# hanseongbugi/ORB_SLAM3_Study_kr

Hardware: AMD Instinct MI355X
Metric: local-BA windows/sec (50 KF, 10k pts, 10 LM iters) + ORB matches/sec; 1/2/4/8 GPU (higher is better)
Workload: dtype f64; 1 GPU; BASELINE.json configs[1]: synthetic stereo local BA, 50 optimisable + 10 fixed KF, 10k landmarks (~75k stereo edges), optimize(10) with the reference's stop rules; windows_per_gpu=512, global_windows=512, streams_per_gpu=2, parallelism=independent windows, w mod 1

## Files before the change

orb_slam3_study_kr_amd/csrc/lba_device.hip:

```cpp
#include <cstdlib>
#include <cstdio>
#include <atomic>
#include <chrono>
#include <thread>
#include "lba_lm_kernels.h"
#include "lba_schur_items.h"
#include "lba_reduce_solve.h"
#include "solve_plan.h"
#include "lba_pack_device.h"
#include <algorithm>
#include <cstring>
#include <vector>

using namespace osh;

namespace osh {

constexpr int kDevicePackMinWindows = 24;

__global__ __launch_bounds__(256) void k_gather_out(BatchView bv, const int* lm_perm, int n_points_total, double* out_pose, double* out_pts,
                                                    const int* pt_win) {
  const int t = blockIdx.x * blockDim.x + threadIdx.x;
  if (t < n_points_total) {
    const int w = pt_win[t];
// ... 26 lines not shown
}

struct osh_lba_ctx {
  int device = 0;
  hipStream_t stream = nullptr;
  void* attach[kAttachCount] = {};
  void (*attach_free[kAttachCount])(void*) = {};
  KernelTimer timer;
  int n_windows = 0;
  PackedBatch pb;
  std::vector<const volatile unsigned char*> stop_ptr;
  bool any_stop = false;
  int solve_nb = 24, solve_W = 0, solve_threads = kSolveThreadsLatency;
  bool solve_big = false;
  DevBuf d_bigV, d_bigz, d_bigfail;
  size_t solve_lds = 0, backsub_lds = 0, lin_lds = 0;
  double upload_pack_ms = 0, upload_copy_ms = 0;
  void (*kp_lin_lm)(BatchView) = nullptr;
  void (*kp_schur_sym)(BatchView, int, int) = nullptr;
  void (*kp_schur_cross)(BatchView, int, int) = nullptr;
  void (*kp_finalize)(BatchView) = nullptr;
  void (*kp_backsub)(BatchView) = nullptr;
  void (*kp_debug_hpl)(BatchView, double*) = nullptr;
  PinBuf h_arena[2], h_out;
  DevBuf d_arena[2], d_ptwin, d_erec;
  DevBuf d_lm, d_pose[2], d_pt[2], d_hcontrib, d_chi_lin, d_dmax_lin, d_contrib, d_ccontrib;
  DevBuf d_Hll, d_bl, d_DL, d_Hpp, d_bp, d_S, d_bs, d_xp, d_chi, d_scale, d_dmaxp, d_nactive, d_out_chi2, d_out_depth, d_stop;
  DevBuf d_out_pose, d_out_pts, d_dbg, d_pose_lo;
  int* h_nactive = nullptr;
  unsigned char* h_stop = nullptr;
  size_t h_stop_cap = 0;
  BatchView bv{};
  bool optimized = false;
  DevPackState dpack;
  int pack_mode = -1;
// ... 68 lines not shown
  } else {
    const int rc = pack_batch(nw, pr, [&](int which, size_t bytes) { return c->h_arena[which].reserve(bytes); }, default_pack_threads(nw), cuts, pb);
    if (rc != OSH_OK) { set_error("%s", pb.msg); return rc; }
  }
  const auto t1 = std::chrono::steady_clock::now();
  if (!on_device) {
    for (int a = 0; a < 2; ++a) {
      OSH_TRY(c->d_arena[a].reserve(pb.arena_bytes[a]));
      OSH_HIP(hipMemcpyAsync(c->d_arena[a].p, pb.arena[a], pb.arena_bytes[a], hipMemcpyHostToDevice, s));
    }
  }
  const size_t NP = pb.NP, NFP = pb.NFP, NL = pb.NL, NOUT = pb.NOUT;

  {
    c->lin_lds = (size_t)LinLds::doubles(std::min(pb.np_max, kLdsPoses)) * sizeof(double);
    int backsub_doubles = 0;
    for (const WinDesc& d : pb.win) backsub_doubles = std::max(backsub_doubles, backsub_lds_doubles(d.P, d.F, backsub_stages(d.P, d.F)));
    c->backsub_lds = (size_t)backsub_doubles * sizeof(double);
    auto knob = [](const char* name) { const char* e = std::getenv(name); return e ? std::atoi(e) : 0; };
    const SolvePlan plan = lba_solve_plan(pb.n_max, nw, knob("OSH_LBA_SOLVE_NB"), knob("OSH_LBA_SOLVE_THREADS"), knob("OSH_LBA_SOLVE_BIG"));
    c->solve_threads = plan.threads;
    c->solve_big = plan.big;
    if (c->solve_big) {
      if (pb.n_max / 6 > kBigMaxPoses) {
        set_error("window with %d optimisable poses: the dense reduced system is limited to %d poses", pb.n_max / 6, kBigMaxPoses);
        return OSH_ERR_UNSUPPORTED;
      }
      OSH_TRY(c->d_bigV.reserve(std::max<size_t>((size_t)kBigNB * pb.n_max * 8, 8))); OSH_TRY(c->d_bigz.reserve(std::max<size_t>((size_t)pb.n_max * 8, 8)));
      OSH_TRY(c->d_bigfail.reserve(sizeof(int)));
    }
// ... 9 lines not shown
  OSH_TRY(R(c->d_hcontrib, pb.n_ccontrib * 27 * 8)); OSH_TRY(R(c->d_chi_lin, pb.n_chunks * 8)); OSH_TRY(R(c->d_dmax_lin, pb.n_chunks * 8));
  OSH_TRY(R(c->d_Hll, NL * 6 * 8)); OSH_TRY(R(c->d_bl, NL * 3 * 8)); OSH_TRY(R(c->d_DL, NL * 9 * 8));
  OSH_TRY(R(c->d_Hpp, NFP * 36 * 8)); OSH_TRY(R(c->d_bp, NFP * 6 * 8)); OSH_TRY(R(c->d_S, pb.S_total * 8));
  OSH_TRY(R(c->d_bs, NFP * 6 * 8)); OSH_TRY(R(c->d_xp, NFP * 6 * 8));
  OSH_TRY(R(c->d_chi, pb.n_chunks * 8)); OSH_TRY(R(c->d_scale, pb.n_chunks * 8));
  OSH_TRY(R(c->d_dmaxp, NFP * 8)); OSH_TRY(R(c->d_nactive, sizeof(int)));
  OSH_TRY(R(c->d_out_chi2, NOUT * 8)); OSH_TRY(R(c->d_out_depth, NOUT)); OSH_TRY(R(c->d_stop, nw));
  OSH_TRY(R(c->d_out_pose, NFP * 7 * 8)); OSH_TRY(R(c->d_out_pts, NL * 3 * 8)); OSH_TRY(R(c->d_ptwin, NL * 4)); OSH_TRY(R(c->d_pose_lo, NFP * 4));
  if (c->h_stop_cap < (size_t)nw) {
    if (c->h_stop) (void)hipHostFree(c->h_stop);
    OSH_HIP(hipHostMalloc((void**)&c->h_stop, nw));
    zero_new_host(c->h_stop, nw);
    c->h_stop_cap = nw;
  }
  OSH_HIP(hipMemsetAsync(c->d_xp.p, 0, std::max<size_t>(NFP * 6 * 8, 8), s));
  if (!on_device) {
    int* h_ptwin = static_cast<int*>(c->h_out.reserve(std::max<size_t>(NL * 4, 8)));
    if (!h_ptwin) { set_error("cannot allocate pinned staging"); return OSH_ERR_DEVICE; }
    for (int w = 0; w < nw; ++w) std::fill(h_ptwin + pb.win[w].pt_off, h_ptwin + pb.win[w].pt_off + pb.win[w].L, w);
    if (NL) OSH_HIP(hipMemcpyAsync(c->d_ptwin.p, h_ptwin, NL * 4, hipMemcpyHostToDevice, s));
  }

  BatchView& bv = c->bv;
  bv.n_windows = nw; bv.n_chunks = (int)pb.n_chunks; bv.n_fposes = (int)NFP;
  bv.win = c->dsec<WinDesc>(PackedBatch::WIN); bv.lm = c->d_lm.as<LmState>(); bv.chunks = c->dsec<Chunk>(PackedBatch::CHUNKS);
  bv.fpose_win = c->dsec<int>(PackedBatch::FPW);
  for (int k = 0; k < 2; ++k) { bv.pose_state[k] = c->d_pose[k].as<double>(); bv.pt_state[k] = c->d_pt[k].as<double>(); }
  bv.pose_cam = c->dsec<double>(PackedBatch::CAM);
  bv.e_pose = c->dsec<int>(PackedBatch::EPOSE); bv.e_point = c->dsec<int>(PackedBatch::EPOINT);
  bv.e_kind = c->dsec<unsigned char>(PackedBatch::EKIND);
// ... 24 lines not shown
  bv.n_active = c->d_nactive.as<int>();
  bv.out_chi2 = c->d_out_chi2.as<double>(); bv.out_depth = c->d_out_depth.as<unsigned char>();
  bv.pose_lo = c->d_pose_lo.as<int>();
  hipLaunchKernelGGL(k_schur_env, dim3((unsigned)nw), dim3(256), 0, s, bv);
  OSH_TRY(launch_check("k_schur_env"));
  if (std::getenv("OSH_LBA_DENSE_SOLVE") || c->solve_big) bv.pose_lo = nullptr;
  else OSH_HIP(hipMemsetAsync(c->d_S.p, 0, std::max<size_t>(pb.S_total * 8, 8), s));
  OSH_HIP(hipStreamSynchronize(s));
  const auto t2 = std::chrono::steady_clock::now();
  c->upload_pack_ms = on_device ? c->dpack.host_ms : std::chrono::duration<double, std::milli>(t1 - t0).count();
  c->upload_copy_ms = (on_device ? c->dpack.device_ms : 0.0) + std::chrono::duration<double, std::milli>(t2 - t1).count();

  const bool f32 = bv.e_rec32 != nullptr;
  if (pb.has_kb8) {
    c->kp_lin_lm = f32 ? k_lin_lm<true, true> : k_lin_lm<true, false>; c->kp_schur_sym = k_schur_fused<true, true>; c->kp_schur_cross = k_schur_fused<false, true>;
    c->kp_finalize = k_finalize<true>;
    c->kp_backsub = f32 ? k_backsub<true, true> : k_backsub<true, false>; c->kp_debug_hpl = k_debug_hpl<true>;
  } else {
    c->kp_lin_lm = f32 ? k_lin_lm<false, true> : k_lin_lm<false, false>; c->kp_schur_cross = k_schur_fused<false, false>;
    c->kp_schur_sym = std::getenv("OSH_LBA_SCHUR_TILES") ? k_schur_fused<true, false> : k_schur_fused<true, false, true>;
    c->kp_finalize = k_finalize<false>;
    c->kp_backsub = f32 ? k_backsub<false, true> : k_backsub<false, false>; c->kp_debug_hpl = k_debug_hpl<false>;
  }

  constexpr int kTB = kSolveThreadsBatch, kTL = kSolveThreadsLatency;
  OSH_TRY(allow_dynamic_lds(c->device, kMaxDynamicLds, k_solve<24, kTB>, k_solve<12, kTB>, k_solve<6, kTB>, k_solve<24, kTL>,
                            k_solve<12, kTL>, k_solve<6, kTL>, k_backsub<false, false>, k_backsub<false, true>, k_backsub<true, false>,
                            k_backsub<true, true>, k_lin_lm<false, false>, k_lin_lm<false, true>, k_lin_lm<true, false>, k_lin_lm<true, true>));
  c->n_windows = nw;
  return OSH_OK;
}

static bool snapshot_stop(osh_lba_ctx* c) {
  bool any = false;
  for (int w = 0; w < c->n_windows; ++w) {
    const volatile unsigned char* f = c->stop_ptr[w];
    c->h_stop[w] = (f && *f) ? 1 : 0;
    any |= c->h_stop[w] != 0;
  }
  return any;
}

#define LAUNCH(kid, name, grid, block, lds, ...)                                              \
// ... 27 lines not shown
      }
      hipLaunchKernelGGL(k_big_back, dim3(1), dim3(1024), 0, s, g);
      hipLaunchKernelGGL(k_big_finish, dim3(1), dim3(256), 0, s, c->bv, w, g.fail);
    }
    return launch_check("k_big_solve");
  }
  const dim3 grid((unsigned)c->n_windows);
#define OSH_SOLVE_CASE(NB, NT) \
  if (c->solve_nb == NB && c->solve_threads == NT) hipLaunchKernelGGL((k_solve<NB, NT>), grid, dim3(NT), c->solve_lds, s, c->bv, c->solve_W);
  OSH_SOLVE_CASE(24, kSolveThreadsBatch) OSH_SOLVE_CASE(12, kSolveThreadsBatch) OSH_SOLVE_CASE(6, kSolveThreadsBatch)
  OSH_SOLVE_CASE(24, kSolveThreadsLatency) OSH_SOLVE_CASE(12, kSolveThreadsLatency) OSH_SOLVE_CASE(6, kSolveThreadsLatency)
#undef OSH_SOLVE_CASE
  return launch_check("k_solve");
}

static int reset_state(osh_lba_ctx* c) {
  hipStream_t s = c->stream;
  const PackedBatch& pb = c->pb;
  for (int k = 0; k < 2; ++k) {
    if (pb.NP) OSH_HIP(hipMemcpyAsync(c->d_pose[k].p, c->dsec<double>(PackedBatch::POSE), pb.NP * 7 * 8, hipMemcpyDeviceToDevice, s));
    if (pb.NL) OSH_HIP(hipMemcpyAsync(c->d_pt[k].p, c->dsec<double>(PackedBatch::PT), pb.NL * 3 * 8, hipMemcpyDeviceToDevice, s));
  }
  OSH_HIP(hipMemsetAsync(c->d_nactive.p, 0, sizeof(int), s));
  const unsigned char* dstop = nullptr;
  if (c->any_stop) {
    snapshot_stop(c);
    OSH_HIP(hipMemcpyAsync(c->d_stop.p, c->h_stop, c->n_windows, hipMemcpyHostToDevice, s));
    dstop = c->d_stop.as<unsigned char>();
  }
  hipLaunchKernelGGL(k_reset, dim3((c->n_windows + 63) / 64), dim3(64), 0, s, c->bv, dstop);
  OSH_TRY(launch_check("k_reset"));
  return OSH_OK;
}

static int read_nactive(osh_lba_ctx* c, int* out) {
  OSH_HIP(hipMemcpyAsync(c->h_nactive, c->d_nactive.p, sizeof(int), hipMemcpyDeviceToHost, c->stream));
  OSH_HIP(hipStreamSynchronize(c->stream));
  *out = *c->h_nactive;
  return OSH_OK;
}

static int first_linearisation(osh_lba_ctx* c) {
  hipStream_t s = c->stream;
  const PackedBatch& pb = c->pb;
  LAUNCH(OSH_K_LINEARIZE, c->kp_lin_lm, pb.n_chunks, kBlock, c->lin_lds, c->bv);
  LAUNCH(OSH_K_LIN_POSE, c->kp_schur_sym, pb.n_sym, 64, 0, c->bv, 0, 0);
  LAUNCH(OSH_K_POSE_HESS, k_pose_reduce, (pb.NFP + 1) / 2, 64, 0, c->bv, 0);
  LAUNCH(OSH_K_CONTROL, k_control, c->n_windows, 64, 0, c->bv, 0);
  LAUNCH(OSH_K_LIN_AUX, c->kp_lin_lm, pb.n_chunks, kBlock, c->lin_lds, c->bv);
  return OSH_OK;
}

static int launch_schur_reduce(osh_lba_ctx* c) {
  hipStream_t s = c->stream;
  const int n = (int)c->pb.n_rblk;
  if (c->n_windows <= 8) { LAUNCH(OSH_K_SCHUR_REDUCE, k_schur_reduce_deep, (n + 6) / 7, 256, 0, c->bv); }
  else { LAUNCH(OSH_K_SCHUR_REDUCE, k_schur_reduce, (n + 13) / 14, 256, 0, c->bv); }
  return OSH_OK;
}

static int trial_kernels(osh_lba_ctx* c, bool later_round) {
// ... 6 lines not shown
  {
    const bool _t = c->timer.begin(OSH_K_SOLVE, s);
    OSH_TRY(launch_solve(c, s));
    if (_t) c->timer.end(s);
  }
  LAUNCH(OSH_K_BACKSUB, c->kp_backsub, pb.n_chunks, kBlock, c->backsub_lds, c->bv);
  return OSH_OK;
}

extern "C" int osh_lba_optimize(osh_lba_ctx* c) {
  if (!c || c->n_windows <= 0) { set_error("osh_lba_optimize: nothing uploaded"); return OSH_ERR_INVALID; }
  OSH_HIP(hipSetDevice(c->device));
  hipStream_t s = c->stream;
  const PackedBatch& pb = c->pb;
  if (c->timer.enabled) OSH_TRY(c->timer.init());
  OSH_TRY(reset_state(c));
  int n_active = 0;
  OSH_TRY(read_nactive(c, &n_active));
  int max_iter = 0;
  for (const WinDesc& d : pb.win) max_iter = std::max(max_iter, d.max_iter);
  const long max_rounds = (long)max_iter * kLmMaxTrials + 1;
  for (long round = 0; round < max_rounds && n_active > 0; ++round) {
    if (round == 0) {
      OSH_TRY(first_linearisation(c));
    } else {
      LAUNCH(OSH_K_LINEARIZE, c->kp_lin_lm, pb.n_chunks, kBlock, c->lin_lds, c->bv);
      LAUNCH(OSH_K_CONTROL, k_control, c->n_windows, 64, 0, c->bv, 0);
    }
    OSH_TRY(trial_kernels(c, round > 0));
    if (c->any_stop) {
      snapshot_stop(c);
      OSH_HIP(hipMemcpyAsync(c->d_stop.p, c->h_stop, c->n_windows, hipMemcpyHostToDevice, s));
      hipLaunchKernelGGL(k_set_stop, dim3((c->n_windows + 63) / 64), dim3(64), 0, s, c->bv, c->d_stop.as<unsigned char>());
      OSH_TRY(launch_check("k_set_stop"));
    }
    LAUNCH(OSH_K_CONTROL, k_control, c->n_windows, 64, 0, c->bv, 1);
    if (c->any_stop || round + 1 >= (long)max_iter) {
      OSH_TRY(read_nactive(c, &n_active));
      if (c->timer.enabled) c->timer.collect();
    }
  }
  if (pb.n_chunks) {
    hipLaunchKernelGGL(c->kp_finalize, dim3((unsigned)pb.n_chunks), dim3(kBlock), 0, s, c->bv);
    OSH_TRY(launch_check("k_finalize"));
  }
  {
    const size_t n = std::max(pb.NL, pb.NFP);
    if (n) {
      hipLaunchKernelGGL(k_gather_out, dim3((unsigned)((n + 255) / 256)), dim3(256), 0, s, c->bv, c->dsec<int>(PackedBatch::LMPERM), (int)pb.NL,
                         c->d_out_pose.as<double>(), c->d_out_pts.as<double>(), c->d_ptwin.as<int>());
      OSH_TRY(launch_check("k_gather_out"));
    }
  }
  OSH_HIP(hipStreamSynchronize(s));
  if (c->timer.enabled) c->timer.collect();
  c->optimized = true;
  return OSH_OK;
}
// ... 52 lines not shown

static int host_ints(osh_lba_ctx* c, int sec, size_t count, std::vector<int>& store, const int*& out) {
  if (!c->device_packed) { out = c->pb.sec<int>(sec); return OSH_OK; }
  store.resize(std::max<size_t>(count, 1));
  if (count) OSH_HIP(hipMemcpy(store.data(), c->dsec<int>(sec), count * 4, hipMemcpyDeviceToHost));
  out = store.data();
  return OSH_OK;
}

extern "C" int osh_lba_linearize(osh_lba_ctx* c, int32_t window, double* Hpp, double* bp, double* Hll, double* bl,
                                 double* Hpl, double* chi2, double* robust_chi2) {
  if (!c || window < 0 || window >= c->n_windows) { set_error("osh_lba_linearize: bad window"); return OSH_ERR_INVALID; }
  OSH_HIP(hipSetDevice(c->device));
  hipStream_t s = c->stream;
  const PackedBatch& pb = c->pb;
  OSH_TRY(reset_state(c));
  OSH_TRY(first_linearisation(c));
  OSH_HIP(hipStreamSynchronize(s));
  const WinDesc& d = pb.win[window];
  std::vector<LmState> h_lm(c->n_windows);
  OSH_HIP(hipMemcpy(h_lm.data(), c->d_lm.p, c->n_windows * sizeof(LmState), hipMemcpyDeviceToHost));
  if (robust_chi2) *robust_chi2 = h_lm[window].chi2_initial;
  if (Hpp && d.P) OSH_HIP(hipMemcpy(Hpp, c->d_Hpp.as<double>() + (size_t)d.fpose_off * 36, (size_t)d.P * 36 * 8, hipMemcpyDeviceToHost));
  if (bp && d.P) OSH_HIP(hipMemcpy(bp, c->d_bp.as<double>() + (size_t)d.fpose_off * 6, (size_t)d.P * 6 * 8, hipMemcpyDeviceToHost));
  std::vector<int> perm_store, eo_store, eo2_store;
  const int* perm = nullptr;
  OSH_TRY(host_ints(c, PackedBatch::LMPERM, pb.NL, perm_store, perm));
  perm += d.pt_off;
  if (bl && d.L) {
    std::vector<double> t((size_t)d.L * 3);
    OSH_HIP(hipMemcpy(t.data(), c->d_bl.as<double>() + (size_t)d.pt_off * 3, t.size() * 8, hipMemcpyDeviceToHost));
// ... 16 lines not shown
    std::vector<double> hs((size_t)d.E * 18);
    if (d.E) OSH_HIP(hipMemcpy(hs.data(), c->d_dbg.as<double>() + (size_t)d.edge_off * 18, hs.size() * 8, hipMemcpyDeviceToHost));
    std::memset(Hpl, 0, (size_t)d.in_edges * 18 * 8);
    const int *eo = nullptr, *eo2 = nullptr;
    OSH_TRY(host_ints(c, PackedBatch::EORIG, pb.NE, eo_store, eo));
    eo += d.edge_off;
    if (pb.has_rig) { OSH_TRY(host_ints(c, PackedBatch::EORIG2, pb.NE, eo2_store, eo2)); eo2 += d.edge_off; }
    for (int x = 0; x < d.E; ++x) {
      std::memcpy(Hpl + (size_t)eo[x] * 18, &hs[(size_t)x * 18], 18 * 8);
      if (eo2 && eo2[x] >= 0) std::memcpy(Hpl + (size_t)eo2[x] * 18, &hs[(size_t)x * 18], 18 * 8);
    }
  }
  if (chi2 && d.in_edges) {
    for (auto& st : h_lm) { st.iterations = 1; st.last_eval_sel = st.sel; }
    OSH_HIP(hipMemcpy(c->d_lm.p, h_lm.data(), c->n_windows * sizeof(LmState), hipMemcpyHostToDevice));
    hipLaunchKernelGGL(c->kp_finalize, dim3((unsigned)pb.n_chunks), dim3(kBlock), 0, s, c->bv);
    OSH_TRY(launch_check("k_finalize"));
    OSH_HIP(hipStreamSynchronize(s));
    OSH_HIP(hipMemcpy(chi2, c->d_out_chi2.as<double>() + d.out_off, (size_t)d.in_edges * 8, hipMemcpyDeviceToHost));
  }
  c->optimized = false;
  return OSH_OK;
}

extern "C" int osh_lba_debug_trial(osh_lba_ctx* c, int32_t window, double lambda, double* S, double* bs, double* x) {
  if (!c || window < 0 || window >= c->n_windows) { set_error("osh_lba_debug_trial: bad window"); return OSH_ERR_INVALID; }
  OSH_HIP(hipSetDevice(c->device));
  hipStream_t s = c->stream;
  const PackedBatch& pb = c->pb;
  OSH_TRY(reset_state(c));
  LAUNCH(OSH_K_LINEARIZE, c->kp_lin_lm, pb.n_chunks, kBlock, c->lin_lds, c->bv);
  LAUNCH(OSH_K_LIN_POSE, c->kp_schur_sym, pb.n_sym, 64, 0, c->bv, 0, 0);
  LAUNCH(OSH_K_POSE_HESS, k_pose_reduce, (pb.NFP + 1) / 2, 64, 0, c->bv, 0);
  LAUNCH(OSH_K_CONTROL, k_control, c->n_windows, 64, 0, c->bv, 0);
  OSH_HIP(hipStreamSynchronize(s));
  std::vector<LmState> h_lm(c->n_windows);
  OSH_HIP(hipMemcpy(h_lm.data(), c->d_lm.p, c->n_windows * sizeof(LmState), hipMemcpyDeviceToHost));
  for (auto& st : h_lm) { st.lambda = lambda; st.need_dl = 1; }
  OSH_HIP(hipMemcpy(c->d_lm.p, h_lm.data(), c->n_windows * sizeof(LmState), hipMemcpyHostToDevice));
  const WinDesc& d = pb.win[window];
  LAUNCH(OSH_K_LIN_AUX, c->kp_lin_lm, pb.n_chunks, kBlock, c->lin_lds, c->bv);
  LAUNCH(OSH_K_SCHUR, c->kp_schur_sym, pb.n_sym, 64, 0, c->bv, 0, 1);
  LAUNCH(OSH_K_SCHUR_CROSS, c->kp_schur_cross, pb.n_items - pb.n_sym, 64, 0, c->bv, (int)pb.n_sym, 1);
  OSH_TRY(launch_schur_reduce(c));
  OSH_HIP(hipStreamSynchronize(s));
  if (S && d.n) OSH_HIP(hipMemcpy(S, c->d_S.as<double>() + d.S_off, (size_t)d.n * d.n * 8, hipMemcpyDeviceToHost));
  if (bs && d.n) OSH_HIP(hipMemcpy(bs, c->d_bs.as<double>() + (size_t)d.fpose_off * 6, (size_t)d.n * 8, hipMemcpyDeviceToHost));
// ... 66 lines not shown
  for (int k = 0; k < 4; ++k) ms[k] = c->dpack.ev_ms[k];
  ms[4] = (double)c->dpack.raw_bytes; ms[5] = c->device_packed ? 1.0 : 0.0;
  for (int k = 0; k < 24; ++k) ms[6 + k] = c->dpack.cyc_mean[k];
  return OSH_OK;
}

extern "C" int osh_lba_get_upload_times(osh_lba_ctx* c, double ms[2]) {
  if (!c || !ms) return OSH_ERR_INVALID;
  ms[0] = c->upload_pack_ms; ms[1] = c->upload_copy_ms;
  return OSH_OK;
}

extern "C" const char* osh_lba_kernel_name(int k) {
  static const char* names[OSH_K_COUNT] = {"k_lin_lm<false, true>", "k_pose_reduce", "k_schur_fused<true, false> (mode 1)", "k_solve", "k_backsub<false, true>",
                                           "k_residual<false, true>", "k_control", "k_schur_reduce", "k_schur_fused<false, false>",
                                           "k_lin_lm<false, true> (factors only)", "k_schur_fused<true, false> (mode 0)"};
  return (k >= 0 && k < OSH_K_COUNT) ? names[k] : "?";
}
```

orb_slam3_study_kr_amd/csrc/lba_lm_kernels.h:

```cpp
#pragma once
#include "lba_chunk.h"

namespace osh {
template <bool KB8, bool F32>
__global__ __launch_bounds__(kBlock) void k_lin_lm(BatchView bv) {
  extern __shared__ __attribute__((aligned(16))) double sh_lm[];
  const Chunk ch = bv.chunks[blockIdx.x];
  const WinDesc wd = bv.win[ch.win];
  const LmView st = lm_view(bv.lm, ch.win);
  if (!st.active || (!st.need_lin && !st.need_dl)) return;
  const int tid = threadIdx.x;
  const int nl = ch.lm1 - ch.lm0;
  const bool lambda_known = st.lambda >= 0.0;
  if (!st.need_lin) {
    if (tid < nl) {
      const size_t gl = (size_t)wd.pt_off + ch.lm0 + tid;
      double hl[6], bl[3], dl[9];
#pragma unroll
      for (int k = 0; k < 6; ++k) hl[k] = bv.Hll[gl * 6 + k];
#pragma unroll
      for (int k = 0; k < 3; ++k) bl[k] = bv.bl[gl * 3 + k];
      dev::landmark_factor(hl, bl, st.lambda, dl);
#pragma unroll
      for (int k = 0; k < 9; ++k) bv.DL[gl * 9 + k] = dl[k];
// ... 193 lines not shown
      if (e < e1) {
        double qt[7], cam[5], R[9], X[3];
        fetch_pose(staged_t, sh_pose_t, poses_t, cams, le.ip[p], qt, cam, R);
#pragma unroll
        for (int k = 0; k < 3; ++k) X[k] = sh_X[(le.il[p] - ch.lm0) * 3 + k];
        const double rec[4] = {le.ra[p].x, le.ra[p].y, le.rb[p].x, le.rb[p].y};
        double cl, cr;
        chi_acc += win_edge_rho<KB8>(wd, bv, (size_t)wd.edge_off + e, rec, qt, cam, R, X, cl, cr);
      }
    }
  }
  const double chi = block_sum(chi_acc, sh4);
  if (tid == 0) bv.chi_part[blockIdx.x] = chi;
}

template <bool KB8>
__global__ __launch_bounds__(kBlock) void k_finalize(BatchView bv) {
  const Chunk ch = bv.chunks[blockIdx.x];
  const WinDesc wd = bv.win[ch.win];
  const LmView st = lm_view(bv.lm, ch.win);
  const int* lmo = bv.lm_off + wd.lmoff_off;
  const int e0 = lmo[ch.lm0], e1 = lmo[ch.lm1];
  const bool evaluated = st.iterations > 0;
  for (int e = e0 + threadIdx.x; e < e1; e += kBlock) {
    const size_t ge = (size_t)wd.edge_off + e;
    const int ip = bv.e_pose[ge], il = bv.e_point[ge];
    double qt[7], cam[5], X[3], rec[4];
#pragma unroll
    for (int k = 0; k < 5; ++k) cam[k] = bv.pose_cam[((size_t)wd.pose_off + ip) * 5 + k];
#pragma unroll
    for (int k = 0; k < 4; ++k) rec[k] = bv.e_rec[ge * 4 + k];
    double chi_l = 0.0, chi_r = 0.0;
// ... 75 lines not shown
```

orb_slam3_study_kr_amd/csrc/lba_reduce_solve.h:

```cpp
#pragma once
#include <cfloat>
#include "lba_view.h"
#include "ldlt_block.h"
#include "big_solve.h"
#include "g2o_lm.h"

namespace osh {

__device__ __forceinline__ void reduce_load8(double2* t, const double* c, int k, int n) {
#pragma unroll
  for (int u = 0; u < 8; ++u)
    if (k + u < n) t[u] = *reinterpret_cast<const double2*>(c + (size_t)k * 36 + u * 36);
}

__global__ __launch_bounds__(256) void k_schur_reduce(BatchView bv) {
  const int t = threadIdx.x / 18, e = threadIdx.x - 18 * t;
  const int idx = blockIdx.x * 14 + t;
  if (t >= 14 || idx >= bv.n_rblk) return;
  const int r = e / 3, cc = 2 * (e - 3 * r);
  const RBlk rb = bv.rblk[idx];
  const WinDesc& wd = bv.win[rb.win];
  const LmState& st = bv.lm[rb.win];
  const int fpose_off = wd.fpose_off, n = wd.n;
  const long long S_off = wd.S_off;
// ... 299 lines not shown
  }
}

__global__ void k_reset(BatchView bv, const unsigned char* stop) {
  const int w = blockIdx.x * blockDim.x + threadIdx.x;
  if (w >= bv.n_windows) return;
  const WinDesc& wd = bv.win[w];
  LmState& st = bv.lm[w];
  st.lambda = -1.0; st.ni = 2.0; st.currentChi = 0; st.iniChi = 0; st.tempChi = 0; st.rho = 0; st.scale_pose = 0;
  st.chi2_initial = 0;
  st.iter = 0; st.qmax = 0; st.nBad = 0;
  st.stop = stop ? stop[w] : 0;
  st.active = (wd.max_iter > 0 && !st.stop && wd.E > 0) ? 1 : 0;
  st.need_lin = st.active; st.lin_now = 0; st.need_dl = 0;
  st.sel = 0; st.last_eval_sel = 0; st.iterations = 0; st.trials = 0; st.solve_ok = 1; st.n_trace = 0;
  if (st.active) atomicAdd(bv.n_active, 1);
}

__global__ void k_set_stop(BatchView bv, const unsigned char* stop) {
  const int w = blockIdx.x * blockDim.x + threadIdx.x;
  if (w >= bv.n_windows) return;
  bv.lm[w].stop = stop[w];
}
}
```

orb_slam3_study_kr_amd/csrc/lba_schur_items.h:

```cpp
#pragma once
#include <type_traits>
#include "lba_chunk.h"

namespace osh {
typedef double f64x4 __attribute__((ext_vector_type(4)));
constexpr int kSiLm = 8;
constexpr int kSiRows = 6 * kItemPoses;
constexpr int kSiImage = 32 * 49;

template <bool SYM, bool KB8, bool BLK = false>
__global__ __launch_bounds__(64, KB8 ? 1 : 2) void k_schur_fused(BatchView bv, int item_base, int mode) {
  static_assert(!BLK || (SYM && !KB8), "block path: symmetric pinhole items");
  __shared__ double shA[(SYM && !KB8) ? kSiImage : kSiRows * (3 * kSiLm + 1)];
  __shared__ double shB[SYM ? 1 : kSiRows * (3 * kSiLm + 1)];
  __shared__ double shPose[(SYM ? 1 : 2) * 8 * kPoseRec];
  __shared__ int shP[64 + 8];
  const int item_idx = item_base + blockIdx.x;
  const SItem it = bv.sitems[item_idx];
  const WinDesc wd = bv.win[it.win];
  const LmView st = lm_view(bv.lm, it.win);
  if (!st.active) return;
  const bool do_hpp = SYM && (mode == 0 ? st.need_lin != 0 : (st.lin_now != 0 && st.iter > 0));
  const bool do_schur = mode != 0;
  if (!do_hpp && !do_schur) return;
  const int lane = threadIdx.x;
  const int nx = it.shape & 0xff, ny = (it.shape >> 8) & 0xff;
  const int TX = (6 * nx + 15) >> 4, TY = (6 * ny + 15) >> 4;
  shP[lane] = bv.spair[(size_t)item_idx * 64 + lane];
  if (lane < 8) shP[64 + lane] = bv.scslot[(size_t)item_idx * 8 + lane];
  {
    const double* poses = bv.pose_state[st.sel] + (size_t)wd.pose_off * 7;
    const double* cams = bv.pose_cam + (size_t)wd.pose_off * 5;
    const int side = lane >> 3, s8 = lane & 7;
    if (side < (SYM ? 1 : 2)) {
      const int ip = side == 0 ? bv.sposex[(size_t)item_idx * 8 + s8] : bv.sposey[(size_t)item_idx * 8 + s8];
      double qt[7], cam[5], Rm[9];
#pragma unroll
      for (int k = 0; k < 7; ++k) qt[k] = ip >= 0 ? poses[(size_t)ip * 7 + k] : 0.0;
#pragma unroll
      for (int k = 0; k < 5; ++k) cam[k] = ip >= 0 ? cams[(size_t)ip * 5 + k] : 0.0;
      dev::quat_to_R(qt, Rm);
      double* dst = shPose + (side * 8 + s8) * kPoseRec;
#pragma unroll
// ... 2 lines not shown
      for (int k = 0; k < 5; ++k) dst[7 + k] = cam[k];
#pragma unroll
      for (int k = 0; k < 9; ++k) dst[12 + k] = Rm[k];
    }
  }
  const SRec* __restrict__ recs = bv.srecs + it.rec_off;
  const double* pts = bv.pt_state[st.sel] + (size_t)wd.pt_off * 3;
  const double* DL = bv.DL + (size_t)wd.pt_off * 9;
  const int mrow = lane & 15, mk = lane >> 4;
  using std::integral_constant;

  auto body = [&](auto lmc, auto psc) __attribute__((always_inline)) {
    constexpr int LM = decltype(lmc)::value, PS = decltype(psc)::value;
    constexpr int KS = 3 * LM + 1;
    constexpr int KST = (3 * LM) / 4;
    static_assert(LM * PS <= 64 && (3 * LM) % 4 == 0 && ((6 * PS + 15) / 16) * 16 * KS <= ((SYM && !KB8) ? kSiImage : kSiRows * (3 * kSiLm + 1)), "chunk mapping");
    const int l = lane / PS, s = lane - l * PS;
    const bool lane_on = LM * PS == 64 || l < LM;
    f64x4 acc[3][3];
#pragma unroll
    for (int a = 0; a < 3; ++a)
#pragma unroll
      for (int b = 0; b < 3; ++b) acc[a][b] = (f64x4){0.0, 0.0, 0.0, 0.0};
    double bacc[3][3][3];
#pragma unroll
    for (int a = 0; a < 3; ++a)
#pragma unroll
      for (int b = 0; b < 3; ++b)
#pragma unroll
        for (int q = 0; q < 3; ++q) bacc[a][b][q] = 0.0;
    double csum[6] = {0, 0, 0, 0, 0, 0};
    double H[21], hb[6];
#pragma unroll
    for (int k = 0; k < 21; ++k) H[k] = 0.0;
#pragma unroll
    for (int k = 0; k < 6; ++k) hb[k] = 0.0;
    if (PS < 8) {
      for (int idx = lane; idx < (((6 * PS + 15) / 16) * 16 - 6 * PS) * KS; idx += 64) shA[6 * PS * KS + idx] = 0.0;
    }

    struct Dat { double2 ex[2]; double2 ey[2]; double X[3]; double dl[9]; };
    const int last_rec = it.n_lm - 1;
    const size_t last_edge = (size_t)wd.edge_off + (size_t)max(wd.E - 1, 0);
    auto load_rec = [&](int c0, int4& ra, int4& rb) {
      const int4* src = reinterpret_cast<const int4*>(recs + min(c0 + l, last_rec));
      ra = src[0]; rb = src[1];
    };
    auto slot_of = [&](unsigned lo, unsigned hi) { return (((s < 4) ? lo : hi) >> (8 * (s & 3))) & 0xffu; };
    auto edge_of = [&](const int4& ra, unsigned o) { return min((size_t)wd.edge_off + (size_t)(ra.y + (o != kAbsent ? (int)o : 0)), last_edge); };
    auto load_dat = [&](const int4& ra, const int4& rb, Dat& d) {
      const double2* src = reinterpret_cast<const double2*>(bv.e_rec + edge_of(ra, slot_of((unsigned)ra.z, (unsigned)ra.w)) * 4);
      d.ex[0] = src[0]; d.ex[1] = src[1];
// ... 411 lines not shown
```

orb_slam3_study_kr_amd/csrc/lba_view.h:

```cpp
#pragma once
#include "common.h"
#include "lba_math.h"
#include "schur_plan.h"
#include "lba_pack.h"

namespace osh {
constexpr int kPoseRec = 21;
constexpr int kLdsPoses = 512;
constexpr int kMaxDynamicLds = 160 * 1024 - 64;
constexpr int kPasses = kChunkMaxEdges / kChunkEdges;

struct LmState {
  double lambda, ni, currentChi, iniChi, tempChi, rho, scale_pose, chi2_initial;
  int iter;
  int qmax;
  int nBad;
  int active;
  int need_lin;
  int lin_now;
  int need_dl;
  int sel;
  int last_eval_sel;
  int iterations;
  int trials;
// ... 78 lines not shown
  __syncthreads();
  return r;
}

__device__ __forceinline__ void wave_sync() {
  __builtin_amdgcn_fence(__ATOMIC_RELEASE, "wavefront");
  __builtin_amdgcn_wave_barrier();
  __builtin_amdgcn_fence(__ATOMIC_ACQUIRE, "wavefront");
}

struct LinLds {
  static constexpr int kPart = 0, kRed = kPart + 9 * kChunkEdges, kX = kRed + 4, kPose = kX + 3 * kBlock;
  __host__ __device__ static constexpr int doubles(int n_staged) { return kPose + n_staged * kPoseRec; }
};

struct BacksubLds {
  static constexpr int kPart = 0, kRed = kPart + 3 * kChunkEdges, kX = kRed + 4, kXp = kX + 3 * kBlock;
  int pose, pose_t, doubles;
  bool staged_t;
  __host__ __device__ static constexpr BacksubLds of(int P, int F, bool staged) {
    const int pose = kXp + (staged ? 6 * P : 0), pose_t = pose + (staged ? P * kPoseRec : 0);
    const bool staged_t = P + F <= kLdsPoses;
    return BacksubLds{pose, pose_t, pose_t + (staged_t ? (P + F) * kPoseRec : 0), staged_t};
  }
};
__host__ __device__ constexpr int backsub_lds_doubles(int P, int F, bool staged) { return BacksubLds::of(P, F, staged).doubles; }
__host__ __device__ constexpr bool backsub_stages(int P, int F) {
  return P <= kLdsPoses && backsub_lds_doubles(P, F, true) * (int)sizeof(double) <= kMaxDynamicLds;
}
static_assert(backsub_stages(50, 10) && backsub_lds_doubles(50, 10, true) == 4150, "the headline window stages everything");
// ... 6 lines not shown
```

Baseline: 15070 windows/s.

## Stage finalize in LDS, add pose-only Schur variant, count active windows on host

Rewrites k_finalize to stage points and poses of both LM states in shared memory and to use f32 edge records where available. Adds a POSE_ONLY instantiation of k_schur_fused for the first linearisation pass, which skips the Schur product setup and uses a smaller shared buffer. reset_state now copies only one pose/point state and computes the active window count on the host instead of through a device atomic and a readback. Together these aim to cut per-call latency and kernel work, at the cost of more template instantiations and a host-side count that must match the device rule.

```diff
diff --git a/orb_slam3_study_kr_amd/csrc/lba_device.hip b/orb_slam3_study_kr_amd/csrc/lba_device.hip
--- a/orb_slam3_study_kr_amd/csrc/lba_device.hip
+++ b/orb_slam3_study_kr_amd/csrc/lba_device.hip
@@ -64,11 +64,12 @@
   int solve_nb = 24, solve_W = 0, solve_threads = kSolveThreadsLatency;
   bool solve_big = false;
   DevBuf d_bigV, d_bigz, d_bigfail;
-  size_t solve_lds = 0, backsub_lds = 0, lin_lds = 0;
+  size_t solve_lds = 0, backsub_lds = 0, lin_lds = 0, fin_lds = 0;
   double upload_pack_ms = 0, upload_copy_ms = 0;
   void (*kp_lin_lm)(BatchView) = nullptr;
   void (*kp_schur_sym)(BatchView, int, int) = nullptr;
   void (*kp_schur_cross)(BatchView, int, int) = nullptr;
+  void (*kp_pose_only)(BatchView, int, int) = nullptr;
   void (*kp_finalize)(BatchView) = nullptr;
   void (*kp_backsub)(BatchView) = nullptr;
   void (*kp_debug_hpl)(BatchView, double*) = nullptr;
@@ -167,6 +168,7 @@
 
   {
     c->lin_lds = (size_t)LinLds::doubles(std::min(pb.np_max, kLdsPoses)) * sizeof(double);
+    c->fin_lds = (size_t)FinLds::doubles(std::min(pb.np_max, kLdsPoses)) * sizeof(double);
     int backsub_doubles = 0;
     for (const WinDesc& d : pb.win) backsub_doubles = std::max(backsub_doubles, backsub_lds_doubles(d.P, d.F, backsub_stages(d.P, d.F)));
     c->backsub_lds = (size_t)backsub_doubles * sizeof(double);
@@ -206,6 +208,7 @@
     c->h_stop_cap = nw;
   }
   OSH_HIP(hipMemsetAsync(c->d_xp.p, 0, std::max<size_t>(NFP * 6 * 8, 8), s));
+  if (NP) OSH_HIP(hipMemcpyAsync(c->d_pose[1].p, c->dsec<double>(PackedBatch::POSE), NP * 7 * 8, hipMemcpyDeviceToDevice, s));
   if (!on_device) {
     int* h_ptwin = static_cast<int*>(c->h_out.reserve(std::max<size_t>(NL * 4, 8)));
     if (!h_ptwin) { set_error("cannot allocate pinned staging"); return OSH_ERR_DEVICE; }
@@ -260,19 +263,22 @@
   const bool f32 = bv.e_rec32 != nullptr;
   if (pb.has_kb8) {
     c->kp_lin_lm = f32 ? k_lin_lm<true, true> : k_lin_lm<true, false>; c->kp_schur_sym = k_schur_fused<true, true>; c->kp_schur_cross = k_schur_fused<false, true>;
-    c->kp_finalize = k_finalize<true>;
+    c->kp_finalize = f32 ? k_finalize<true, true> : k_finalize<true, false>; c->kp_pose_only = k_schur_fused<true, true, false, true>;
     c->kp_backsub = f32 ? k_backsub<true, true> : k_backsub<true, false>; c->kp_debug_hpl = k_debug_hpl<true>;
   } else {
     c->kp_lin_lm = f32 ? k_lin_lm<false, true> : k_lin_lm<false, false>; c->kp_schur_cross = k_schur_fused<false, false>;
     c->kp_schur_sym = std::getenv("OSH_LBA_SCHUR_TILES") ? k_schur_fused<true, false> : k_schur_fused<true, false, true>;
-    c->kp_finalize = k_finalize<false>;
+    c->kp_finalize = f32 ? k_finalize<false, true> : k_finalize<false, false>; c->kp_pose_only = k_schur_fused<true, false, false, true>;
     c->kp_backsub = f32 ? k_backsub<false, true> : k_backsub<false, false>; c->kp_debug_hpl = k_debug_hpl<false>;
   }
+  if (std::getenv("OSH_LBA_POSE_PASS_FULL")) c->kp_pose_only = c->kp_schur_sym;
+  if (std::getenv("OSH_LBA_FINALIZE_PLAIN")) { c->kp_finalize = pb.has_kb8 ? k_finalize_plain<true> : k_finalize_plain<false>; c->fin_lds = 0; }
 
   constexpr int kTB = kSolveThreadsBatch, kTL = kSolveThreadsLatency;
   OSH_TRY(allow_dynamic_lds(c->device, kMaxDynamicLds, k_solve<24, kTB>, k_solve<12, kTB>, k_solve<6, kTB>, k_solve<24, kTL>,
                             k_solve<12, kTL>, k_solve<6, kTL>, k_backsub<false, false>, k_backsub<false, true>, k_backsub<true, false>,
-                            k_backsub<true, true>, k_lin_lm<false, false>, k_lin_lm<false, true>, k_lin_lm<true, false>, k_lin_lm<true, true>));
+                            k_backsub<true, true>, k_lin_lm<false, false>, k_lin_lm<false, true>, k_lin_lm<true, false>, k_lin_lm<true, true>,
+                            k_finalize<false, false>, k_finalize<false, true>, k_finalize<true, false>, k_finalize<true, true>));
   c->n_windows = nw;
   return OSH_OK;
 }
@@ -330,14 +336,13 @@
   return launch_check("k_solve");
 }
 
-static int reset_state(osh_lba_ctx* c) {
+static int reset_state(osh_lba_ctx* c, int* n_active, bool both = false) {
   hipStream_t s = c->stream;
   const PackedBatch& pb = c->pb;
-  for (int k = 0; k < 2; ++k) {
+  for (int k = 0; k < (both ? 2 : 1); ++k) {
     if (pb.NP) OSH_HIP(hipMemcpyAsync(c->d_pose[k].p, c->dsec<double>(PackedBatch::POSE), pb.NP * 7 * 8, hipMemcpyDeviceToDevice, s));
     if (pb.NL) OSH_HIP(hipMemcpyAsync(c->d_pt[k].p, c->dsec<double>(PackedBatch::PT), pb.NL * 3 * 8, hipMemcpyDeviceToDevice, s));
   }
-  OSH_HIP(hipMemsetAsync(c->d_nactive.p, 0, sizeof(int), s));
   const unsigned char* dstop = nullptr;
   if (c->any_stop) {
     snapshot_stop(c);
@@ -346,6 +351,10 @@
   }
   hipLaunchKernelGGL(k_reset, dim3((c->n_windows + 63) / 64), dim3(64), 0, s, c->bv, dstop);
   OSH_TRY(launch_check("k_reset"));
+  int n = 0;
+  for (int w = 0; w < c->n_windows; ++w) n += (pb.win[w].max_iter > 0 && !(c->any_stop && c->h_stop[w]) && pb.win[w].E > 0) ? 1 : 0;
+  if (n_active) *n_active = n;
+  if (c->any_stop) OSH_HIP(hipStreamSynchronize(s));
   return OSH_OK;
 }
 
@@ -360,7 +369,7 @@
   hipStream_t s = c->stream;
   const PackedBatch& pb = c->pb;
   LAUNCH(OSH_K_LINEARIZE, c->kp_lin_lm, pb.n_chunks, kBlock, c->lin_lds, c->bv);
-  LAUNCH(OSH_K_LIN_POSE, c->kp_schur_sym, pb.n_sym, 64, 0, c->bv, 0, 0);
+  LAUNCH(OSH_K_LIN_POSE, c->kp_pose_only, pb.n_sym, 64, 0, c->bv, 0, 0);
   LAUNCH(OSH_K_POSE_HESS, k_pose_reduce, (pb.NFP + 1) / 2, 64, 0, c->bv, 0);
   LAUNCH(OSH_K_CONTROL, k_control, c->n_windows, 64, 0, c->bv, 0);
   LAUNCH(OSH_K_LIN_AUX, c->kp_lin_lm, pb.n_chunks, kBlock, c->lin_lds, c->bv);
@@ -397,9 +406,8 @@
   hipStream_t s = c->stream;
   const PackedBatch& pb = c->pb;
   if (c->timer.enabled) OSH_TRY(c->timer.init());
-  OSH_TRY(reset_state(c));
   int n_active = 0;
-  OSH_TRY(read_nactive(c, &n_active));
+  OSH_TRY(reset_state(c, &n_active));
   int max_iter = 0;
   for (const WinDesc& d : pb.win) max_iter = std::max(max_iter, d.max_iter);
   const long max_rounds = (long)max_iter * kLmMaxTrials + 1;
@@ -424,7 +432,7 @@
     }
   }
   if (pb.n_chunks) {
-    hipLaunchKernelGGL(c->kp_finalize, dim3((unsigned)pb.n_chunks), dim3(kBlock), 0, s, c->bv);
+    hipLaunchKernelGGL(c->kp_finalize, dim3((unsigned)pb.n_chunks), dim3(kBlock), c->fin_lds, s, c->bv);
     OSH_TRY(launch_check("k_finalize"));
   }
   {
@@ -507,7 +515,7 @@
   OSH_HIP(hipSetDevice(c->device));
   hipStream_t s = c->stream;
   const PackedBatch& pb = c->pb;
-  OSH_TRY(reset_state(c));
+  OSH_TRY(reset_state(c, nullptr, true));
   OSH_TRY(first_linearisation(c));
   OSH_HIP(hipStreamSynchronize(s));
   const WinDesc& d = pb.win[window];
@@ -554,7 +562,7 @@
   if (chi2 && d.in_edges) {
     for (auto& st : h_lm) { st.iterations = 1; st.last_eval_sel = st.sel; }
     OSH_HIP(hipMemcpy(c->d_lm.p, h_lm.data(), c->n_windows * sizeof(LmState), hipMemcpyHostToDevice));
-    hipLaunchKernelGGL(c->kp_finalize, dim3((unsigned)pb.n_chunks), dim3(kBlock), 0, s, c->bv);
+    hipLaunchKernelGGL(c->kp_finalize, dim3((unsigned)pb.n_chunks), dim3(kBlock), c->fin_lds, s, c->bv);
     OSH_TRY(launch_check("k_finalize"));
     OSH_HIP(hipStreamSynchronize(s));
     OSH_HIP(hipMemcpy(chi2, c->d_out_chi2.as<double>() + d.out_off, (size_t)d.in_edges * 8, hipMemcpyDeviceToHost));
@@ -568,9 +576,9 @@
   OSH_HIP(hipSetDevice(c->device));
   hipStream_t s = c->stream;
   const PackedBatch& pb = c->pb;
-  OSH_TRY(reset_state(c));
+  OSH_TRY(reset_state(c, nullptr, true));
   LAUNCH(OSH_K_LINEARIZE, c->kp_lin_lm, pb.n_chunks, kBlock, c->lin_lds, c->bv);
-  LAUNCH(OSH_K_LIN_POSE, c->kp_schur_sym, pb.n_sym, 64, 0, c->bv, 0, 0);
+  LAUNCH(OSH_K_LIN_POSE, c->kp_pose_only, pb.n_sym, 64, 0, c->bv, 0, 0);
   LAUNCH(OSH_K_POSE_HESS, k_pose_reduce, (pb.NFP + 1) / 2, 64, 0, c->bv, 0);
   LAUNCH(OSH_K_CONTROL, k_control, c->n_windows, 64, 0, c->bv, 0);
   OSH_HIP(hipStreamSynchronize(s));
@@ -667,6 +675,6 @@
 extern "C" const char* osh_lba_kernel_name(int k) {
   static const char* names[OSH_K_COUNT] = {"k_lin_lm<false, true>", "k_pose_reduce", "k_schur_fused<true, false> (mode 1)", "k_solve", "k_backsub<false, true>",
                                            "k_residual<false, true>", "k_control", "k_schur_reduce", "k_schur_fused<false, false>",
-                                           "k_lin_lm<false, true> (factors only)", "k_schur_fused<true, false> (mode 0)"};
+                                           "k_lin_lm<false, true> (factors only)", "k_schur_fused<true, false, false, true> (pose side alone)"};
   return (k >= 0 && k < OSH_K_COUNT) ? names[k] : "?";
 }
diff --git a/orb_slam3_study_kr_amd/csrc/lba_lm_kernels.h b/orb_slam3_study_kr_amd/csrc/lba_lm_kernels.h
--- a/orb_slam3_study_kr_amd/csrc/lba_lm_kernels.h
+++ b/orb_slam3_study_kr_amd/csrc/lba_lm_kernels.h
@@ -231,8 +231,98 @@
   if (tid == 0) bv.chi_part[blockIdx.x] = chi;
 }
 
+template <bool KB8, bool F32>
+__global__ __launch_bounds__(kBlock) void k_finalize(BatchView bv) {
+  extern __shared__ __attribute__((aligned(16))) double sh_fin[];
+  const Chunk ch = bv.chunks[blockIdx.x];
+  const WinDesc wd = bv.win[ch.win];
+  const LmView st = lm_view(bv.lm, ch.win);
+  const int tid = threadIdx.x;
+  const int nl = ch.lm1 - ch.lm0;
+  const int* lmo = bv.lm_off + wd.lmoff_off;
+  const int e0 = lmo[ch.lm0], e1 = lmo[ch.lm1];
+  const bool evaluated = st.iterations > 0;
+  const int f = st.sel, s = evaluated ? st.last_eval_sel : f;
+  const bool two = s != f;
+  const int np = wd.P + wd.F;
+  const bool staged = np <= kLdsPoses;
+  double* sh_X = sh_fin + FinLds::kX;
+  double* sh_Xf = two ? sh_fin + FinLds::kXf : sh_X;
+  double* sh_pose = sh_fin + FinLds::kPose;
+  double* sh_qf = sh_pose + np * kPoseRec;
+  const double* poses = bv.pose_state[s] + (size_t)wd.pose_off * 7;
+  const double* poses_f = bv.pose_state[f] + (size_t)wd.pose_off * 7;
+  const double* cams = bv.pose_cam + (size_t)wd.pose_off * 5;
+  const bool rig = KB8 && wd.kb8_on;
+  for (int base = e0; base < e1; base += kChunkMaxEdges) {
+    LaneEdges le;
+    load_lane_edges<F32>(bv, wd, base, e1, tid, le);
+    int eo[kPasses], ek[kPasses];
+#pragma unroll
+    for (int p = 0; p < kPasses; ++p) {
+      const size_t ge = (size_t)wd.edge_off + min(base + p * kChunkEdges + tid, max(e1 - 1, 0));
+      eo[p] = bv.e_orig[ge];
+      ek[p] = rig ? bv.e_kind[ge] : kKindMono;
+    }
+    if (base == e0) {
+      stage_points(sh_X, bv.pt_state[s] + (size_t)wd.pt_off * 3, ch.lm0, nl, tid);
+      if (two) stage_points(sh_Xf, bv.pt_state[f] + (size_t)wd.pt_off * 3, ch.lm0, nl, tid);
+      if (staged) {
+        stage_poses(sh_pose, poses, cams, np, tid, kBlock);
+        if (two) { for (int k = tid; k < 7 * np; k += kBlock) sh_qf[k] = poses_f[k]; }
+      }
+      __syncthreads();
+    }
+#pragma unroll
+    for (int p = 0; p < kPasses; ++p) {
+      const int e = base + p * kChunkEdges + tid;
+      if (e >= e1) continue;
+      const size_t ge = (size_t)wd.edge_off + e;
+      const int ip = le.ip[p], li = le.il[p] - ch.lm0;
+      double qt[7], cam[5], R[9], X[3];
+      fetch_pose(staged, sh_pose, poses, cams, ip, qt, cam, R);
+#pragma unroll
+      for (int k = 0; k < 3; ++k) X[k] = sh_X[li * 3 + k];
+      double chi_l = 0.0, chi_r = 0.0;
+      if (evaluated) {
+        const double rec[4] = {le.ra[p].x, le.ra[p].y, le.rb[p].x, le.rb[p].y};
+        (void)win_edge_rho<KB8>(wd, bv, ge, rec, qt, cam, R, X, chi_l, chi_r);
+      }
+      if (two) {
+#pragma unroll
+        for (int k = 0; k < 7; ++k) qt[k] = staged ? sh_qf[ip * 7 + k] : poses_f[(size_t)ip * 7 + k];
+#pragma unroll
+        for (int k = 0; k < 3; ++k) X[k] = sh_Xf[li * 3 + k];
+      }
+      double rot[3];
+      dev::quat_rotate(qt, X, rot);
+      const double Xl[3] = {rot[0] + qt[4], rot[1] + qt[5], rot[2] + qt[6]};
+      const size_t go = (size_t)wd.out_off + eo[p];
+      const int kind = ek[p];
+      double zr = 0.0;
+      if (KB8 && kind >= kKindBody) {
+        double Xr[3];
+        dev::quat_rotate(wd.trl, Xl, Xr);
+        zr = Xr[2] + wd.trl[6];
+      }
+      if (kind == kKindBody) {
+        bv.out_chi2[go] = chi_r;
+        bv.out_depth[go] = zr > 0.0 ? 1 : 0;
+      } else {
+        bv.out_chi2[go] = chi_l;
+        bv.out_depth[go] = (Xl[2] > 0.0) ? 1 : 0;
+        if (kind == kKindBoth) {
+          const size_t go2 = (size_t)wd.out_off + bv.e_orig2[ge];
+          bv.out_chi2[go2] = chi_r;
+          bv.out_depth[go2] = zr > 0.0 ? 1 : 0;
+        }
+      }
+    }
+  }
+}
+
 template <bool KB8>
-__global__ __launch_bounds__(kBlock) void k_finalize(BatchView bv) {
+__global__ __launch_bounds__(kBlock) void k_finalize_plain(BatchView bv) {
   const Chunk ch = bv.chunks[blockIdx.x];
   const WinDesc wd = bv.win[ch.win];
   const LmView st = lm_view(bv.lm, ch.win);
diff --git a/orb_slam3_study_kr_amd/csrc/lba_reduce_solve.h b/orb_slam3_study_kr_amd/csrc/lba_reduce_solve.h
--- a/orb_slam3_study_kr_amd/csrc/lba_reduce_solve.h
+++ b/orb_slam3_study_kr_amd/csrc/lba_reduce_solve.h
@@ -337,7 +337,6 @@
   st.active = (wd.max_iter > 0 && !st.stop && wd.E > 0) ? 1 : 0;
   st.need_lin = st.active; st.lin_now = 0; st.need_dl = 0;
   st.sel = 0; st.last_eval_sel = 0; st.iterations = 0; st.trials = 0; st.solve_ok = 1; st.n_trace = 0;
-  if (st.active) atomicAdd(bv.n_active, 1);
 }
 
 __global__ void k_set_stop(BatchView bv, const unsigned char* stop) {
diff --git a/orb_slam3_study_kr_amd/csrc/lba_schur_items.h b/orb_slam3_study_kr_amd/csrc/lba_schur_items.h
--- a/orb_slam3_study_kr_amd/csrc/lba_schur_items.h
+++ b/orb_slam3_study_kr_amd/csrc/lba_schur_items.h
@@ -8,10 +8,16 @@
 constexpr int kSiRows = 6 * kItemPoses;
 constexpr int kSiImage = 32 * 49;
 
-template <bool SYM, bool KB8, bool BLK = false>
+constexpr int kSiPoseRed = 14 * 64;
+
+template <bool SYM, bool KB8, bool BLK = false, bool POSE_ONLY = false>
 __global__ __launch_bounds__(64, KB8 ? 1 : 2) void k_schur_fused(BatchView bv, int item_base, int mode) {
   static_assert(!BLK || (SYM && !KB8), "block path: symmetric pinhole items");
-  __shared__ double shA[(SYM && !KB8) ? kSiImage : kSiRows * (3 * kSiLm + 1)];
+  static_assert(!POSE_ONLY || (SYM && !BLK), "pose side alone: symmetric items, no products");
+  constexpr bool kSchur = !POSE_ONLY;
+  constexpr int kImage = POSE_ONLY ? kSiPoseRed : ((SYM && !KB8) ? kSiImage : kSiRows * (3 * kSiLm + 1));
+  static_assert(kImage >= kSiPoseRed, "the lane reduction of the pose side goes through the image buffer");
+  __shared__ double shA[kImage];
   __shared__ double shB[SYM ? 1 : kSiRows * (3 * kSiLm + 1)];
   __shared__ double shPose[(SYM ? 1 : 2) * 8 * kPoseRec];
   __shared__ int shP[64 + 8];
@@ -21,12 +27,12 @@
   const LmView st = lm_view(bv.lm, it.win);
   if (!st.active) return;
   const bool do_hpp = SYM && (mode == 0 ? st.need_lin != 0 : (st.lin_now != 0 && st.iter > 0));
-  const bool do_schur = mode != 0;
+  const bool do_schur = kSchur && mode != 0;
   if (!do_hpp && !do_schur) return;
   const int lane = threadIdx.x;
   const int nx = it.shape & 0xff, ny = (it.shape >> 8) & 0xff;
   const int TX = (6 * nx + 15) >> 4, TY = (6 * ny + 15) >> 4;
-  shP[lane] = bv.spair[(size_t)item_idx * 64 + lane];
+  if (kSchur) shP[lane] = bv.spair[(size_t)item_idx * 64 + lane];
   if (lane < 8) shP[64 + lane] = bv.scslot[(size_t)item_idx * 8 + lane];
   {
     const double* poses = bv.pose_state[st.sel] + (size_t)wd.pose_off * 7;
@@ -59,7 +65,7 @@
     constexpr int LM = decltype(lmc)::value, PS = decltype(psc)::value;
     constexpr int KS = 3 * LM + 1;
     constexpr int KST = (3 * LM) / 4;
-    static_assert(LM * PS <= 64 && (3 * LM) % 4 == 0 && ((6 * PS + 15) / 16) * 16 * KS <= ((SYM && !KB8) ? kSiImage : kSiRows * (3 * kSiLm + 1)), "chunk mapping");
+    static_assert(LM * PS <= 64 && (3 * LM) % 4 == 0 && (POSE_ONLY || ((6 * PS + 15) / 16) * 16 * KS <= kImage), "chunk mapping");
     const int l = lane / PS, s = lane - l * PS;
     const bool lane_on = LM * PS == 64 || l < LM;
     f64x4 acc[3][3];
@@ -80,7 +86,7 @@
     for (int k = 0; k < 21; ++k) H[k] = 0.0;
 #pragma unroll
     for (int k = 0; k < 6; ++k) hb[k] = 0.0;
-    if (PS < 8) {
+    if (kSchur && PS < 8) {
       for (int idx = lane; idx < (((6 * PS + 15) / 16) * 16 - 6 * PS) * KS; idx += 64) shA[6 * PS * KS + idx] = 0.0;
     }
 
diff --git a/orb_slam3_study_kr_amd/csrc/lba_view.h b/orb_slam3_study_kr_amd/csrc/lba_view.h
--- a/orb_slam3_study_kr_amd/csrc/lba_view.h
+++ b/orb_slam3_study_kr_amd/csrc/lba_view.h
@@ -116,6 +116,12 @@
   __host__ __device__ static constexpr int doubles(int n_staged) { return kPose + n_staged * kPoseRec; }
 };
 
+struct FinLds {
+  static constexpr int kX = 0, kXf = kX + 3 * kBlock, kPose = kXf + 3 * kBlock;
+  __host__ __device__ static constexpr int doubles(int n_staged) { return kPose + n_staged * (kPoseRec + 7); }
+};
+static_assert(FinLds::doubles(kLdsPoses) * (int)sizeof(double) <= kMaxDynamicLds, "kLdsPoses keyframes of both states fit the block");
+
 struct BacksubLds {
   static constexpr int kPart = 0, kRed = kPart + 3 * kChunkEdges, kX = kRed + 4, kXp = kX + 3 * kBlock;
   int pose, pose_t, doubles;
```

After: 15440 windows/s (median of 6 runs). +2.5%, better.
